# g1mv/density

Measured on NVIDIA H100. Metric: chameleon_encode_input_GBps, higher is better.
Workload: dtype u32

## Files before the change

### density_b200/csrc/chameleon_encode.cu

```cuda
#include <cstdio>
#include "common.cuh"
#include "encode_internal.cuh"

namespace dns {
namespace cham {

constexpr int TILE_Q = 4096;
__device__ __forceinline__ bool bit_test(const uint32_t* bm, uint32_t i) { return (bm[i >> 5] >> (i & 31)) & 1u; }

constexpr int F6_THREADS = 512, F6_QPT = 8;
constexpr int F6_NW = F6_THREADS / 32, F6_WQ = 32 * F6_QPT;
static_assert(F6_THREADS * F6_QPT == TILE_Q, "tile geometry");
constexpr int F6_MB_SLOTS = 4096, F6_MB_CAP = 4;
constexpr int F6_SEC_SLOTS = 64, F6_SEC_CAP = 16;
#ifdef DNS_PHASE_TIMING
__device__ long long g_f6_ph[8];
#define F6_PH(k) { if (threadIdx.x == 0 && blockIdx.x == 77) { long long tn = clock64(); g_f6_ph[k] += tn - f6_tprev; f6_tprev = tn; } }
#define F6_PH_DECL long long f6_tprev = clock64();
#else
#define F6_PH(k)
#define F6_PH_DECL
#endif
constexpr uint32_t F6_TOUCHED = 1u << 12, F6_DROPPED = 1u << 13;
struct Flag6Smem {
// ... 211 lines not shown
                const uint32_t n = (S.mbcnt[buf][slot >> 2] >> ((slot & 3u) * 8u)) & 0xFFu;
                const uint2 e2 = *reinterpret_cast<const uint2*>(&S.mb[slot][0]);
                const uint32_t me = ((hh >> 12) << 12) | myidx;
                int best = -1;
#pragma unroll
                for (int t = 0; t < F6_MB_CAP; ++t) {
                    const uint32_t e = ((t & 2) ? e2.y : e2.x) >> ((t & 1) * 16) & 0xFFFFu;
                    if ((uint32_t)t < n && ((e ^ me) >> 12) == 0) {
                        if (e < me) best = max(best, (int)(e & 0xFFFu));
                        later |= e > me;
                    }
                }
                if (n > (uint32_t)F6_MB_CAP) {
                    const uint32_t s2 = slot & (F6_SEC_SLOTS - 1);
                    const uint32_t n2 = S.seccnt[buf][s2];
                    const uint32_t mine = (hh << 12) | myidx;
                    #pragma unroll 1
                    for (uint32_t t4 = 0; t4 < n2; t4 += 4) {
                        const uint4 e4 = *reinterpret_cast<const uint4*>(&S.sec[s2][t4]);
                        const uint32_t ev[4] = {e4.x, e4.y, e4.z, e4.w};
#pragma unroll
                        for (int t = 0; t < 4; ++t) {
                            const uint32_t e = ev[t];
                            if (t4 + t < n2 && ((e ^ mine) & 0xFFFFF000u) == 0) {
                                if (e < mine) best = max(best, (int)(e & 0xFFFu));
                                later |= e > mine;
                            }
                        }
                    }
                }
                if (best >= 0) hit = (S.rec[best].x >> 16) == ff;
                else if (r.y & F6_TOUCHED) hit = (r.y >> 16) == ff;
                else unres = true;
                if (!later) {
                    S.tab[hh] = (uint16_t)ff;
                    if (ff == 0) atomicOr(&S.vbit[hh >> 5], 1u << (hh & 31));
                }
                if (hit) atomicOr(&S.sigw[buf][pos >> 5], 1u << (pos & 31));
            }
            f6_append_unres(unres, run_q0 + pos, r.x, &S.unres_count, unres_run);
        }
    }
    __syncthreads();
    F6_PH(3)
}

__global__ void __launch_bounds__(F6_THREADS, 1)
cham_flag_pass6(const uint32_t* __restrict__ in, uint64_t nquads, uint32_t tiles_total, uint32_t nruns,
                uint32_t* __restrict__ sigw_g, uint2* __restrict__ unres, uint32_t* __restrict__ unres_count,
                uint32_t* __restrict__ final_tab, const uint8_t* __restrict__ copymap, const Status* __restrict__ gate)
{
    if (gate && !(gate->nonquiet && !gate->converged)) return;
    extern __shared__ __align__(16) unsigned char smem_raw[];
    Flag6Smem& S = *reinterpret_cast<Flag6Smem*>(smem_raw);
    const uint32_t tid = threadIdx.x, lane = tid & 31, warp = tid >> 5;
    const uint32_t run = blockIdx.x;
    const uint64_t t_begin = (uint64_t)run * tiles_total / nruns;
    const uint64_t t_end = (uint64_t)(run + 1) * tiles_total / nruns;
    uint2* __restrict__ unres_run = unres + (size_t)run * 65536;
    const uint32_t pos0 = warp * F6_WQ + lane;
    const uint32_t ntile_run = (uint32_t)(t_end - t_begin);
    const uint64_t q_begin = t_begin * TILE_Q;
    const uint64_t q_end64 = (t_end * TILE_Q < nquads) ? t_end * TILE_Q : nquads;
    const uint32_t run_quads = q_begin < q_end64 ? (uint32_t)(q_end64 - q_begin) : 0u;
    const uint32_t* __restrict__ rin = in + q_begin;
    uint32_t* __restrict__ rsig = sigw_g + t_begin * (TILE_Q / 32);
    const uint8_t* __restrict__ rcm = copymap ? copymap + t_begin * 64 : nullptr;
    {
        const uint4 z = make_uint4(0, 0, 0, 0);
        uint4* t4 = reinterpret_cast<uint4*>(S.tab);
        #pragma unroll 1
        for (uint32_t i = tid; i < 65536 * 2 / 16; i += F6_THREADS) t4[i] = z;
        #pragma unroll 1
        for (uint32_t i = tid; i < 2048; i += F6_THREADS) S.vbit[i] = 0;
        #pragma unroll 1
        for (uint32_t i = tid; i < F6_MB_SLOTS / 4; i += F6_THREADS) { S.mbcnt[0][i] = 0; S.mbcnt[1][i] = 0; }
        if (tid < F6_SEC_SLOTS) { S.seccnt[0][tid] = 0; S.seccnt[1][tid] = 0; }
        if (tid == 0) { S.unres_count = 0; S.overflow = 0; }
    }
    __syncthreads();
    uint32_t nxt[F6_QPT], nxt2[F6_QPT];
#pragma unroll
    for (int j = 0; j < F6_QPT; ++j) {
        nxt[j] = (pos0 + 32 * j < run_quads) ? ld_stream_u32(rin + pos0 + 32 * j) : 0u;
        nxt2[j] = (TILE_Q + pos0 + 32 * j < run_quads) ? ld_stream_u32(rin + TILE_Q + pos0 + 32 * j) : 0u;
    }
    #pragma unroll 1
    for (uint32_t lt = 0; lt < ntile_run; ++lt) {
        uint32_t q[F6_QPT];
        const uint32_t run_q0 = lt * TILE_Q;
        const uint32_t left = run_q0 < run_quads ? run_quads - run_q0 : 0u;
        const uint32_t buf = lt & 1u;
#pragma unroll
        for (int j = 0; j < F6_QPT; ++j) { q[j] = nxt[j]; nxt[j] = nxt2[j]; }
        {
            const uint32_t nleft = left > 2u * TILE_Q ? left - 2u * TILE_Q : 0u;
            const uint32_t* __restrict__ np = rin + run_q0 + 2 * TILE_Q + pos0;
            if (nleft >= (uint32_t)TILE_Q) {
#pragma unroll
                for (int j = 0; j < F6_QPT; ++j) nxt2[j] = ld_stream_u32(np + 32 * j);
            } else {
#pragma unroll
                for (int j = 0; j < F6_QPT; ++j) nxt2[j] = (pos0 + 32 * j < nleft) ? ld_stream_u32(np + 32 * j) : 0u;
            }
        }
        if (left >= (uint32_t)TILE_Q && !rcm) {
            f6_tile<false>(S, q, (1u << F6_QPT) - 1u, buf, run_q0, unres_run);
        } else {
            uint32_t validmask = 0, cp = 0;
            if (rcm) {
#pragma unroll
                for (int b = 0; b < F6_WQ / 64; ++b) cp |= (rcm[lt * 64 + warp * (F6_WQ / 64) + b] ? 1u : 0u) << b;
            }
#pragma unroll
            for (int j = 0; j < F6_QPT; ++j)
                if (pos0 + 32 * j < left && !((cp >> (j >> 1)) & 1u)) validmask |= 1u << j;
            f6_tile<true>(S, q, validmask, buf, run_q0, unres_run);
        }
        if (tid < TILE_Q / 32) rsig[lt * (TILE_Q / 32) + tid] = S.sigw[buf][tid];
        if (tid == 0) S.overflow = 0;
    }
    #pragma unroll 1
    for (uint32_t i = tid; i < 65536; i += F6_THREADS) {
        const uint32_t v = S.tab[i];
        const uint32_t tch = (v != 0 || bit_test(S.vbit, i)) ? 0x10000u : 0u;
        final_tab[(size_t)run * 65536 + i] = v | tch;
    }
    if (tid == 0) unres_count[run] = S.unres_count < 65536u ? S.unres_count : 65536u;
#ifdef DNS_PHASE_TIMING
    if (tid == 0 && run == 77 && ntile_run) { const long long nt = ntile_run;
        printf("f6 run %u tiles %lld cycles/tile: A %lld B %lld C+deposit %lld D+S4 %lld  overflow tiles %lld dirty/tile %lld\n", run, nt, g_f6_ph[0] / nt, g_f6_ph[1] / nt,
               g_f6_ph[2] / nt, g_f6_ph[3] / nt, g_f6_ph[6], g_f6_ph[7] / nt);
        for (int k = 0; k < 8; ++k) g_f6_ph[k] = 0; }
#endif
}

__device__ __forceinline__ bool gate_open(const Status* g) { return !g || (g->nonquiet && !g->converged); }

__global__ void cham_carry_scan(const uint32_t* __restrict__ final_tab, const uint32_t* __restrict__ init, int init_untouched,
                                uint32_t nruns, uint32_t* __restrict__ carry, uint32_t* __restrict__ table_out,
                                const Status* __restrict__ gate = nullptr) {
    if (!gate_open(gate)) return;
    uint32_t hb = blockIdx.x * blockDim.x + threadIdx.x;
    if (hb >= 65536) return;
    uint32_t c = init ? init[hb] : ((hb == 0 && !init_untouched) ? 0x10000u : 0u);
    for (uint32_t r = 0; r < nruns; ++r) {
        if (carry) carry[(size_t)r * 65536 + hb] = c;
        uint32_t v = final_tab[(size_t)r * 65536 + hb];
        if (v & 0x10000u) c = v;
    }
    if (table_out) table_out[hb] = c;
}

__global__ void cham_resolve(const uint2* __restrict__ unres, const uint32_t* __restrict__ unres_count,
                             const uint32_t* __restrict__ carry, uint32_t tiles_total, uint32_t nruns,
                             uint32_t* __restrict__ sigw_g, const Status* __restrict__ gate = nullptr) {
    if (!gate_open(gate)) return;
    const uint32_t run = blockIdx.y;
    const uint32_t n = unres_count[run];
    const uint64_t run_q0 = ((uint64_t)run * tiles_total / nruns) * TILE_Q;
    for (uint32_t i = blockIdx.x * blockDim.x + threadIdx.x; i < n; i += gridDim.x * blockDim.x) {
        uint2 e = unres[(size_t)run * 65536 + i];
        uint32_t c = carry[(size_t)run * 65536 + (e.y & 0xFFFFu)];
        if ((c & 0x10000u) && (c & 0xFFFFu) == (e.y >> 16)) {
            uint64_t gq = run_q0 + e.x;
            atomicOr(&sigw_g[gq >> 5], 1u << (gq & 31));
        }
    }
}

struct ProtSmem {
    uint16_t tab[65536];
    uint32_t vbit[2048];
};

__global__ void __launch_bounds__(1024, 1)
cham_protected_pass(const uint32_t* __restrict__ in, uint64_t nbytes, const Status* __restrict__ status, int only_if_nonquiet,
                    uint32_t* __restrict__ sigw_g, uint8_t* __restrict__ copymap) {
    if (only_if_nonquiet && !(status->nonquiet && !status->converged)) return;
    extern __shared__ __align__(16) unsigned char smem_raw[];
    ProtSmem& S = *reinterpret_cast<ProtSmem*>(smem_raw);
    const uint32_t tid = threadIdx.x, lane = tid & 31;
    {
        uint4 z = make_uint4(0, 0, 0, 0);
        uint4* t4 = reinterpret_cast<uint4*>(S.tab);
        for (uint32_t i = tid; i < 65536 * 2 / 16; i += blockDim.x) t4[i] = z;
        for (uint32_t i = tid; i < 2048; i += blockDim.x) S.vbit[i] = (i == 0) ? 1u : 0u;
    }
    __syncthreads();
    if (tid >= 32) return;

    const uint64_t nquads = nbytes / 4;
    const uint64_t nblocks = (nbytes + 255) / 256;
    Protection ps; ps.init();
    uint32_t n0 = 0, n1 = 0;
    if (nblocks) {
        if (lane < nquads) n0 = in[lane];
        if (32 + lane < nquads) n1 = in[32 + lane];
    }
    for (uint64_t b = 0; b < nblocks; ++b) {
        const uint32_t q0 = n0, q1 = n1;
        {
            uint64_t g = (b + 1) * 64 + lane;
            n0 = (b + 1 < nblocks && g < nquads) ? in[g] : 0u;
            n1 = (b + 1 < nblocks && g + 32 < nquads) ? in[g + 32] : 0u;
        }
        const uint64_t bq0 = b * 64;
        const uint32_t nq = (uint32_t)((nquads - bq0 < 64) ? (nquads - bq0) : 64);
        if (ps.revert_to_copy()) {
            if (lane == 0) { copymap[b] = 1; sigw_g[2 * b] = 0; sigw_g[2 * b + 1] = 0; }
            ps.decay();
            continue;
        }
        uint32_t sig[2];
#pragma unroll
        for (int half = 0; half < 2; ++half) {
            const uint32_t q = half ? q1 : q0;
            const bool valid = half * 32 + lane < nq;
            const uint32_t p = hash_prod(q);
            uint32_t hh = valid ? prod_hash(p) : 0x10000u + lane;
            const uint32_t ff = prod_fp(p, q);
            uint32_t cur = 0; bool touched = false;
            if (valid) { cur = S.tab[hh]; touched = cur != 0 || bit_test(S.vbit, hh); }
            const uint32_t grp = __match_any_sync(0xFFFFFFFFu, hh);
            const uint32_t lower = grp & lanemask_lt();
            const int pl = lower ? 31 - __clz(lower) : 0;
            const uint32_t fprev = __shfl_sync(0xFFFFFFFFu, ff, pl);
            const bool hit = valid && (lower ? (fprev == ff) : (touched && cur == ff));
            const bool is_last = (grp & lanemask_gt()) == 0;
            if (valid && is_last && (lower || !hit)) {
                S.tab[hh] = (uint16_t)ff;
                if (ff == 0) atomicOr(&S.vbit[hh >> 5], 1u << (hh & 31));
            }
            sig[half] = __ballot_sync(0xFFFFFFFFu, hit);
            __syncwarp();
        }
        if (lane == 0) { copymap[b] = 0; sigw_g[2 * b] = sig[0]; sigw_g[2 * b + 1] = sig[1]; }
        const uint32_t hits = __popc(sig[0]) + __popc(sig[1]);
        const uint32_t tailb = (b == nblocks - 1) ? (uint32_t)(nbytes & 3) : 0u;
        const uint32_t out_sz = 8 + 4 * nq - 2 * hits + tailb;
        ps.update(out_sz >= 256);
    }
}

constexpr int PSEG = 256;

__device__ __forceinline__ uint32_t prot_pack(const Protection& ps) { return ps.copy_penalty | (ps.copy_penalty_start << 8) | (ps.previous_incompressible << 16); }
__device__ __forceinline__ void prot_walk(Protection& ps, const uint8_t* __restrict__ inc, uint64_t b0, uint64_t b1, uint8_t* __restrict__ cm) {
    for (uint64_t b = b0; b < b1; ++b) {
        if (ps.revert_to_copy()) { cm[b] = 1; ps.decay(); }
        else { cm[b] = 0; ps.update(__ldcg(&inc[b]) != 0); }
    }
}
constexpr int PROT_ROUNDS = 48, PROT_FAST_ROUNDS = 4;
constexpr int PI_THREADS = 1024;

constexpr uint32_t PC_NS = 10, PC_NP = 10, PC_NC = 2 * PC_NS * PC_NP, PC_ESC = 0xFFFFu, PC_GROUP = 128;
__host__ __device__ __forceinline__ size_t prot_table_elems(uint64_t nseg) {
    const uint64_t ngrp = (nseg + PC_GROUP - 1) / PC_GROUP;
    return (size_t)(2 * (ngrp + 2) + nseg * PC_NC + ngrp * PC_NC + 64);
}
__device__ __forceinline__ void pc_decode(uint32_t c, Protection& ps) {
    ps.copy_penalty = c % PC_NP; ps.copy_penalty_start = (c / PC_NP) % PC_NS + 1u; ps.previous_incompressible = c / (PC_NP * PC_NS);
}
__device__ __forceinline__ uint32_t pc_encode(const Protection& ps) {
    if (ps.copy_penalty >= PC_NP || ps.copy_penalty_start < 1u || ps.copy_penalty_start > PC_NS) return PC_ESC;
    return (ps.previous_incompressible * PC_NS + (ps.copy_penalty_start - 1u)) * PC_NP + ps.copy_penalty;
}

__device__ __forceinline__ void grid_barrier(unsigned int* counter, unsigned int nctas, unsigned int& epoch) {
    __syncthreads();
    if (threadIdx.x == 0) {
        __threadfence();
        atomicAdd(counter, 1u);
        const unsigned int target = (epoch + 1) * nctas;
        while (atomicAdd(counter, 0u) < target) { __nanosleep(64); }
        __threadfence();
    }
    ++epoch;
    __syncthreads();
}

__device__ unsigned long long g_prot_dbg[16][2];

__global__ void __launch_bounds__(PI_THREADS)
prot_iterate(const uint32_t* __restrict__ sigw_g, uint64_t nbytes, uint64_t nblocks, uint32_t nseg, Status* __restrict__ st, int it,
             uint8_t* __restrict__ inc, uint8_t* __restrict__ cm_old, uint8_t* __restrict__ cm_new,
             uint32_t* __restrict__ in_state, uint32_t* __restrict__ out_state, uint16_t* __restrict__ ptab) {
    if (!gate_open(st)) return;
    __shared__ uint32_t s_state[1024], s_in[1024];
    __shared__ uint8_t s_inc[PSEG], s_cm[PSEG];
    __shared__ uint32_t s_cur, s_redo;
    const uint32_t tid = threadIdx.x;
    const uint64_t gtid = (uint64_t)blockIdx.x * PI_THREADS + tid, gsz = (uint64_t)gridDim.x * PI_THREADS;
    unsigned int epoch = 0;
    unsigned int* bar = &st->barrier[it & 7];

    if (sigw_g)
        for (uint64_t b = gtid; b < nblocks; b += gsz)
            if (!(it && cm_old[b])) inc[b] = (nbytes - b * 256 >= 256) && (__popc(sigw_g[2 * b]) + __popc(sigw_g[2 * b + 1]) <= 4);
    if (gtid == 0) { st->relax_changed[0] = 0; st->relax_changed[1] = 0; st->iter_changed = 0; st->pad2[0] = 0; }
    if (gtid < 16 && it == 0) { g_prot_dbg[gtid][0] = ~0ull; g_prot_dbg[gtid][1] = 0; }
    grid_barrier(bar, gridDim.x, epoch);

    bool settled = false;
    int round = 0;
    for (int phase = 0; phase < 2 && !settled; ++phase) {
    const int limit = (phase == 0 && ptab) ? PROT_FAST_ROUNDS : PROT_ROUNDS;
    for (; round < limit; ++round) {
        for (uint64_t s = gtid; s < nseg; s += gsz) {
            const uint32_t new_in = (s && round) ? __ldcg(&out_state[s - 1]) : (1u << 8);
            if (round > 0 && new_in == in_state[s]) continue;
            Protection ps;
            ps.copy_penalty = new_in & 0xFFu; ps.copy_penalty_start = (new_in >> 8) & 0xFFu; ps.previous_incompressible = (new_in >> 16) & 1u;
            ps.counter = s * PSEG;
            const uint64_t b1 = ((s + 1) * PSEG < nblocks) ? (s + 1) * PSEG : nblocks;
            prot_walk(ps, inc, s * PSEG, b1, cm_new);
            in_state[s] = new_in;
            out_state[s] = prot_pack(ps);
// ... 494 lines not shown
    while (k < nb) {
        const uint32_t k1 = (k + 16 < nb) ? k + 16 : nb;
        for (; k < k1; ++k) { if (p.revert_to_copy()) p.decay(); else p.update(s_inc[k] != 0); }
        if (tid == 0) s_ref = prot_pack(p);
        __syncthreads();
        if (__syncthreads_and(prot_pack(p) == s_ref)) break;
    }
    if (k < nb) {
        if (tid == 0) {
            for (; k < nb; ++k) { if (p.revert_to_copy()) p.decay(); else p.update(s_inc[k] != 0); }
            s_ref = pc_encode(p);
        }
        __syncthreads();
        if (tid < PC_NC) T[(size_t)seg * PC_NC + tid] = (uint16_t)s_ref;
    } else if (tid < PC_NC) {
        T[(size_t)seg * PC_NC + tid] = (uint16_t)pc_encode(p);
    }
    __syncthreads();
    }
}

__global__ void cham_prot_groups_k(uint32_t nseg, const Status* __restrict__ st, const uint16_t* __restrict__ T, uint16_t* __restrict__ GT) {
    if (!gate_open(st)) return;
    const uint32_t ngrp = (nseg + PC_GROUP - 1) / PC_GROUP;
    const uint64_t idx = (uint64_t)blockIdx.x * blockDim.x + threadIdx.x;
    if (idx >= (uint64_t)ngrp * PC_NC) return;
    const uint32_t g = (uint32_t)(idx / PC_NC);
    uint32_t x = (uint32_t)(idx % PC_NC);
    const uint32_t s1 = ((g + 1) * PC_GROUP < nseg) ? (g + 1) * PC_GROUP : nseg;
    for (uint32_t s = g * PC_GROUP; s < s1 && x != PC_ESC; ++s) x = T[(size_t)s * PC_NC + x];
    GT[idx] = (uint16_t)x;
}
__global__ void cham_prot_transfer_k(uint32_t nseg, const Status* __restrict__ st, const uint16_t* __restrict__ GT, uint32_t* __restrict__ out) {
    if (!gate_open(st)) return;
    const uint32_t c = threadIdx.x;
    if (c >= PC_NC) return;
    const uint32_t ngrp = (nseg + PC_GROUP - 1) / PC_GROUP;
    uint32_t x = c;
    for (uint32_t g = 0; g < ngrp && x != PC_ESC; ++g) x = GT[(size_t)g * PC_NC + x];
    out[c] = x;
}

__global__ void cham_prot_enter_k(const uint32_t* __restrict__ all_transfers, uint32_t rank, uint32_t nseg, const Status* __restrict__ st,
                                  const uint16_t* __restrict__ GT, uint32_t* __restrict__ gin, ProtShard* __restrict__ ps,
                                  uint32_t* __restrict__ words) {
    if (threadIdx.x || blockIdx.x) return;
    const bool open = gate_open(st);
    words[0] = 0; words[1] = 0; words[2] = open ? 0u : 1u; words[3] = 0;
    if (!open) return;
    uint32_t x = 0;
    for (uint32_t r = 0; r < rank && x != PC_ESC; ++r) x = all_transfers[(size_t)r * PC_NC + x];
    ps->in_state = x;
    const uint32_t ngrp = (nseg + PC_GROUP - 1) / PC_GROUP;
    for (uint32_t g = 0; g < ngrp; ++g) { gin[g] = x; if (x != PC_ESC) x = GT[(size_t)g * PC_NC + x]; }
    gin[ngrp] = x;
    if (x == PC_ESC) words[1] = 1;
}
__global__ void cham_prot_seams_k(uint32_t nseg, const Status* __restrict__ st, const uint16_t* __restrict__ T, const uint32_t* __restrict__ gin,
                                  uint32_t* __restrict__ in_state) {
    if (!gate_open(st)) return;
    const uint32_t ngrp = (nseg + PC_GROUP - 1) / PC_GROUP;
    const uint32_t g = blockIdx.x * blockDim.x + threadIdx.x;
    if (g >= ngrp || gin[ngrp] == PC_ESC) return;
    uint32_t x = gin[g];
    const uint32_t s1 = ((g + 1) * PC_GROUP < nseg) ? (g + 1) * PC_GROUP : nseg;
    for (uint32_t s = g * PC_GROUP; s < s1; ++s) { in_state[s] = x; x = T[(size_t)s * PC_NC + x]; }
}
__global__ void cham_prot_walk_k(uint64_t nblocks, uint32_t nseg, const Status* __restrict__ st, int it, int warm, const uint8_t* __restrict__ inc,
                                 const uint8_t* __restrict__ cm_old, uint8_t* __restrict__ cm_new, const uint32_t* __restrict__ in_state,
                                 const uint32_t* __restrict__ gin, ProtShard* __restrict__ ps, uint32_t* __restrict__ words) {
    if (!gate_open(st)) return;
    const uint32_t ngrp = (nseg + PC_GROUP - 1) / PC_GROUP;
    const uint32_t s = blockIdx.x * blockDim.x + threadIdx.x;
    if (s >= nseg || gin[ngrp] == PC_ESC) return;
    Protection p; pc_decode(in_state[s], p);
    const uint64_t b0 = (uint64_t)s * PSEG, b1 = (b0 + PSEG < nblocks) ? b0 + PSEG : nblocks;
    p.counter = ps->first_block + b0;
    prot_walk(p, inc, b0, b1, cm_new);
    uint32_t nd = 0;
    for (uint64_t b = b0; b < b1; ++b) nd += cm_new[b] != ((it || warm) ? cm_old[b] : 0);
    if (nd) {
        atomicAdd(&words[0], nd);
        if (it < 16) atomicAdd(&ps->changed[it], nd);
    }
}

__device__ __forceinline__ void prot_round_verdict(const uint32_t* all_words, uint32_t world, uint32_t stride, bool& changed, bool& esc) {
    changed = false; esc = false;
    for (uint32_t r = 0; r < world; ++r) { changed |= all_words[stride * r] != 0; esc |= all_words[stride * r + 1] != 0; }
}
__global__ void cham_prot_commit_k(const uint32_t* __restrict__ all_words, uint32_t world, uint32_t stride, uint64_t nblocks, const Status* __restrict__ st,
                                   int it, uint8_t* __restrict__ cm_old, const uint8_t* __restrict__ cm_new) {
    if (!gate_open(st)) return;
    bool changed, esc;
    prot_round_verdict(all_words, world, stride, changed, esc);
    if (esc || !(changed || it == 0)) return;
    for (uint64_t b = (uint64_t)blockIdx.x * blockDim.x + threadIdx.x; b < nblocks; b += (uint64_t)gridDim.x * blockDim.x) cm_old[b] = cm_new[b];
}
__global__ void cham_prot_verdict_k(const uint32_t* __restrict__ all_words, uint32_t world, uint32_t stride, Status* __restrict__ st, int it,
                                    ProtShard* __restrict__ ps) {
    if (threadIdx.x || blockIdx.x || !gate_open(st)) return;
    bool changed, esc;
    prot_round_verdict(all_words, world, stride, changed, esc);
    if (esc) { ps->esc = 1; st->converged = 1; }
    else if (!changed) { ps->settled = 1; ps->rounds = (uint32_t)it + 1; st->converged = 1; }
}
__global__ void cham_prot_finish_k(Status* __restrict__ st, const ProtShard* __restrict__ ps) {
    if (threadIdx.x || blockIdx.x) return;
    if (!ps->settled || !ps->stage_ok) st->error = PROT_REFUSED;
}
__global__ void cham_prot_seam_words_k(uint64_t nblocks, const Status* __restrict__ st, uint64_t* __restrict__ d_out_size, uint32_t* __restrict__ words) {
    if (threadIdx.x || blockIdx.x) return;
    const uint64_t sz = (nblocks && !st->error) ? *d_out_size : 0;
    *d_out_size = sz;
    words[0] = 0; words[1] = 0; words[2] = st->error ? 1u : 0u; words[3] = nblocks ? 1u : 0u;
    words[4] = (uint32_t)sz; words[5] = (uint32_t)(sz >> 32); words[6] = 0; words[7] = 0;
}

}

using namespace cham;

size_t cham_workspace_bytes(size_t nbytes, int nruns_max, ChamLayout* L) {
    const uint64_t nblocks = (nbytes + 255) / 256;
    const uint64_t ntiles = (nblocks + 63) / 64;
    const uint64_t ngroups = (ntiles + SCAN_G - 1) / SCAN_G;
    size_t off = 0;
    auto take = [&](size_t bytes) { size_t o = off; off += (bytes + 255) & ~(size_t)255; return o; };
    L->status = take(sizeof(Status));
    L->sigw = take((ntiles * 64 * 2 + 64 + 256) * sizeof(uint32_t));
    L->copymap = take(ntiles * 64 + 64 + 128);
    L->copymap2 = take(ntiles * 64 + 64 + 128);
    L->seg_state = take(prot_state_bytes(ntiles * 64 / PSEG + 2));
    L->incb = take(ntiles * 64 + 64);
    L->tile_bytes = take((ntiles + 1) * sizeof(uint32_t));
    L->tile_local = take((ntiles + 1) * sizeof(uint32_t));
    L->group_total = take((ngroups + 1) * sizeof(uint64_t));
    L->group_off = take((ngroups + 1) * sizeof(uint64_t));
    L->unres = take((size_t)nruns_max * 65536 * sizeof(uint2));
    L->unres_count = take((size_t)nruns_max * sizeof(uint32_t));
    L->final_tab = take((size_t)nruns_max * 65536 * sizeof(uint32_t));
    L->carry = take((size_t)nruns_max * 65536 * sizeof(uint32_t));
    L->total = off;
    return off;
}

static cudaError_t set_smem_attrs_once() {
    static bool done = false;
    static cudaError_t err = cudaSuccess;
    if (!done) {
        err = cudaFuncSetAttribute(cham_flag_pass6, cudaFuncAttributeMaxDynamicSharedMemorySize, (int)sizeof(Flag6Smem));
        if (err == cudaSuccess)
            err = cudaFuncSetAttribute(cham_protected_pass, cudaFuncAttributeMaxDynamicSharedMemorySize, (int)sizeof(ProtSmem));
        done = true;
    }
    return err;
}

static cudaError_t prot_iterate_coop(int ctas, cudaStream_t stream, const uint32_t* sigw, uint64_t nbytes, uint64_t nblocks, uint32_t nseg, Status* st, int it,
                                     uint8_t* inc, uint8_t* cm_old, uint8_t* cm_new, uint32_t* in_state, uint32_t* out_state, uint16_t* ptab) {
    void* args[] = {&sigw, &nbytes, &nblocks, &nseg, &st, &it, &inc, &cm_old, &cm_new, &in_state, &out_state, &ptab};
    return cudaLaunchCooperativeKernel(reinterpret_cast<const void*>(prot_iterate), dim3((unsigned)ctas), dim3(PI_THREADS), args, 0, stream);
}

cudaError_t prot_debug_read(unsigned long long* out32) { return cudaMemcpyFromSymbol(out32, g_prot_dbg, sizeof(unsigned long long) * 32); }

size_t prot_state_bytes(uint64_t nseg_max) { return (2 * (nseg_max + 2) + 64) * sizeof(uint32_t) + prot_table_elems(nseg_max) * sizeof(uint16_t); }

uint32_t cham_pick_runs(size_t nbytes, int num_sms) {
    const uint64_t nblocks = (nbytes + 255) / 256;
    const uint64_t ntiles = (nblocks + 63) / 64;
    uint64_t r = ntiles / 16;
    if (r < 1) r = 1;
    if (r > (uint64_t)num_sms) r = num_sms;
    return (uint32_t)r;
}

struct ChamBufs {
    size_t nbytes; uint64_t nquads, nblocks; uint32_t ntiles, ngroups, nseg, ngrp;
    Status* st; uint32_t* sigw; uint8_t *copymap, *copymap2, *incb; uint32_t *seg_state, *tile_bytes, *tile_local; uint64_t *group_total, *group_off;
    uint2* unres; uint32_t *unres_count, *final_tab, *carry;
    uint32_t *in_state, *out_state, *gin; uint16_t *ptab, *T, *GT;
    template <class X> static X* at(uint8_t* ws, size_t off) { return reinterpret_cast<X*>(ws + off); }
    ChamBufs(uint8_t* ws, const ChamLayout& L, size_t n) {
        nbytes = n; nquads = n / 4; nblocks = (n + 255) / 256;
        ntiles = (uint32_t)((nblocks + 63) / 64); ngroups = (ntiles + SCAN_G - 1) / SCAN_G;
        nseg = (uint32_t)((nblocks + PSEG - 1) / PSEG); ngrp = (nseg + PC_GROUP - 1) / PC_GROUP;
        st = at<Status>(ws, L.status); sigw = at<uint32_t>(ws, L.sigw);
        copymap = ws + L.copymap; copymap2 = ws + L.copymap2; incb = ws + L.incb;
        seg_state = at<uint32_t>(ws, L.seg_state);
        tile_bytes = at<uint32_t>(ws, L.tile_bytes); tile_local = at<uint32_t>(ws, L.tile_local);
        group_total = at<uint64_t>(ws, L.group_total); group_off = at<uint64_t>(ws, L.group_off);
        unres = at<uint2>(ws, L.unres); unres_count = at<uint32_t>(ws, L.unres_count);
        final_tab = at<uint32_t>(ws, L.final_tab); carry = at<uint32_t>(ws, L.carry);
        in_state = seg_state; out_state = seg_state + (nseg + 1);
        ptab = reinterpret_cast<uint16_t*>(seg_state + 2 * (nseg + 1));
        gin = reinterpret_cast<uint32_t*>(ptab); T = ptab + 2 * (ngrp + 2); GT = T + (size_t)nseg * PC_NC;
    }
};

static void launch_flag_pass(const ChamBufs& B, const uint8_t* d_in, uint32_t nruns, const uint8_t* copymap, const Status* gate, cudaStream_t stream,
                             uint64_t* launches) {
    cham_flag_pass6<<<nruns, F6_THREADS, sizeof(Flag6Smem), stream>>>(reinterpret_cast<const uint32_t*>(d_in), B.nquads, B.ntiles, nruns, B.sigw, B.unres,
                                                                      B.unres_count, B.final_tab, copymap, gate);
    ++*launches;
}
static void launch_carry_resolve(const ChamBufs& B, uint32_t nruns, const uint32_t* d_carry_in, const Status* gate, cudaStream_t stream,
                                 uint64_t* launches) {
    cham_carry_scan<<<65536 / 256, 256, 0, stream>>>(B.final_tab, d_carry_in, 0, nruns, B.carry, nullptr, gate);
    cham_resolve<<<dim3(32, nruns), 256, 0, stream>>>(B.unres, B.unres_count, B.carry, B.ntiles, nruns, B.sigw, gate);
    *launches += 2;
}
static void launch_export_fold(const ChamBufs& B, uint32_t nruns, uint32_t* d_table_out, const Status* gate, cudaStream_t stream, uint64_t* launches) {
    cham_carry_scan<<<65536 / 256, 256, 0, stream>>>(B.final_tab, nullptr, 1, nruns, nullptr, d_table_out, gate);
    ++*launches;
}
static cudaError_t sizes_scan_emit(const ChamBufs& B, const uint8_t* d_in, const uint8_t* copymap, int use_copymap_if_nonquiet, bool al16_ok,
                                   uint8_t* d_out, size_t cap, uint64_t* d_out_size, cudaStream_t stream, uint64_t* launches, cudaEvent_t* ev) {
    if (copymap) {
        cham_tile_sizes<<<(B.ntiles + 7) / 8, 256, 0, stream>>>(B.sigw, copymap, B.nbytes, B.nblocks, B.ntiles, use_copymap_if_nonquiet, 0, 0, B.st, B.tile_bytes);
        ++*launches;
    }
    cudaError_t e = scan_tiles_launch(B.tile_bytes, B.ntiles, B.tile_local, B.group_total, B.group_off, B.ngroups, B.st, (uint64_t)cap, d_out_size, stream);
    if (e != cudaSuccess) return e;
    *launches += 2;
    if (ev) cudaEventRecord(ev[2], stream);
    const uint32_t* in32 = reinterpret_cast<const uint32_t*>(d_in);
    if (al16_ok && (reinterpret_cast<uintptr_t>(d_in) & 15u) == 0)
        cham_emit<true><<<B.ntiles, EM_THREADS, 0, stream>>>(in32, B.nbytes, B.nblocks, B.sigw, copymap, use_copymap_if_nonquiet, B.st, B.tile_local, B.group_off, d_out);
    else
        cham_emit<false><<<B.ntiles, EM_THREADS, 0, stream>>>(in32, B.nbytes, B.nblocks, B.sigw, copymap, use_copymap_if_nonquiet, B.st, B.tile_local, B.group_off, d_out);
    ++*launches;
    if (ev) cudaEventRecord(ev[3], stream);
    return cudaGetLastError();
}

cudaError_t cham_encode_phase1(const uint8_t* d_in, size_t nbytes, uint8_t* ws, const ChamLayout& L, uint32_t nruns,
                               uint32_t* d_table_out, cudaStream_t stream, uint64_t* launches, cudaEvent_t* ev) {
    cudaError_t e = set_smem_attrs_once();
    if (e != cudaSuccess) return e;
    const ChamBufs B(ws, L, nbytes);
    e = cudaMemsetAsync(B.st, 0, sizeof(Status), stream);
    if (e == cudaSuccess) e = cudaMemsetAsync(&B.st->first_nonquiet_block, 0xFF, sizeof(unsigned long long), stream);
    if (e != cudaSuccess) return e;
    if (B.nblocks == 0) return cudaSuccess;
    if (ev) cudaEventRecord(ev[0], stream);
    launch_flag_pass(B, d_in, nruns, nullptr, nullptr, stream, launches);
    if (ev) cudaEventRecord(ev[1], stream);
    if (d_table_out) launch_export_fold(B, nruns, d_table_out, nullptr, stream, launches);
    return cudaGetLastError();
}

static cudaError_t cham_phase2_begin(const ChamBufs& B, uint32_t nruns, const uint32_t* d_carry_in, bool assume_prev_inc, cudaStream_t stream,
                                     uint64_t* launches) {
    launch_carry_resolve(B, nruns, d_carry_in, nullptr, stream, launches);
    cham_tile_sizes<<<(B.ntiles + 7) / 8, 256, 0, stream>>>(B.sigw, nullptr, B.nbytes, B.nblocks, B.ntiles, 0, 1, assume_prev_inc ? 1 : 0, B.st, B.tile_bytes);
    ++*launches;
    return cudaGetLastError();
}

static cudaError_t cham_phase2_rounds(const ChamBufs& B, const uint8_t* d_in, uint32_t nruns, const uint32_t* d_carry_in, int it_first, int it_last,
                                      bool reset_barriers, int num_sms, cudaStream_t stream, uint64_t* launches) {
    const int num_ctas = num_sms > 0 ? num_sms : 1;
    if (it_last - it_first >= 8) return cudaErrorInvalidValue;
    if (reset_barriers) {
        cudaError_t e = cudaMemsetAsync(B.st->barrier, 0, sizeof(B.st->barrier), stream);
        if (e != cudaSuccess) return e;
    }
    for (int it = it_first; it <= it_last; ++it) {
        if (it > 0) {
            launch_flag_pass(B, d_in, nruns, B.copymap, B.st, stream, launches);
            launch_carry_resolve(B, nruns, d_carry_in, B.st, stream, launches);
        }
        cudaError_t le = prot_iterate_coop(num_ctas, stream, B.sigw, B.nbytes, B.nblocks, B.nseg, B.st, it, B.incb, B.copymap, B.copymap2, B.in_state,
                                           B.out_state, B.ptab);
        if (le != cudaSuccess) return le;
        ++*launches;
    }
    return cudaGetLastError();
}

static cudaError_t cham_phase2_finish(const ChamBufs& B, const uint8_t* d_in, uint8_t* d_out, size_t cap, uint64_t* d_out_size, bool with_copy_map,
                                      bool inorder_fallback, cudaStream_t stream, uint64_t* launches, cudaEvent_t* ev) {
    if (with_copy_map && inorder_fallback) {
        cham_protected_pass<<<1, 1024, sizeof(ProtSmem), stream>>>(reinterpret_cast<const uint32_t*>(d_in), B.nbytes, B.st, 1, B.sigw, B.copymap);
        ++*launches;
    }
    return sizes_scan_emit(B, d_in, with_copy_map ? B.copymap : nullptr, 1, true, d_out, cap, d_out_size, stream, launches, ev);
}

static cudaError_t cham_phase2_needs_more(const ChamBufs& B, cudaStream_t stream, bool* more) {
    Status h;
    cudaError_t e = cudaMemcpyAsync(&h, B.st, sizeof h, cudaMemcpyDeviceToHost, stream);
    if (e == cudaSuccess) e = cudaStreamSynchronize(stream);
    if (e != cudaSuccess) return e;
    *more = h.nonquiet && !h.converged && !h.error;
    return cudaSuccess;
}

constexpr int PROT_ITERS = 4;

struct Phase2Opts {
    const uint32_t* d_carry_in = nullptr;
    bool assume_prev_inc = false;
    bool iterate = true;
    int max_batches = 0;
    bool inorder_walk = true;
    bool* give_up = nullptr;
    uint32_t* d_table_out = nullptr;
    cudaEvent_t* ev = nullptr;
};

static cudaError_t cham_phase2(const uint8_t* d_in, size_t nbytes, uint8_t* ws, const ChamLayout& L, uint32_t nruns, uint8_t* d_out, size_t cap,
                               uint64_t* d_out_size, const Phase2Opts& o, int num_sms, cudaStream_t stream, uint64_t* launches) {
    if (nbytes == 0) return cudaMemsetAsync(d_out_size, 0, sizeof(uint64_t), stream);
    const ChamBufs B(ws, L, nbytes);
    cudaError_t e = cham_phase2_begin(B, nruns, o.d_carry_in, o.assume_prev_inc, stream, launches);
    if (e == cudaSuccess && o.iterate) e = cham_phase2_rounds(B, d_in, nruns, o.d_carry_in, 0, PROT_ITERS, false, num_sms, stream, launches);
    bool more = false;
    const int looks = o.max_batches + (o.give_up ? 1 : 0);
    for (int batch = 0; e == cudaSuccess && batch < looks; ++batch) {
        e = cham_phase2_needs_more(B, stream, &more);
        if (e != cudaSuccess || !more || batch >= o.max_batches) break;
        e = cham_phase2_rounds(B, d_in, nruns, o.d_carry_in, 8, 15, true, num_sms, stream, launches);
    }
    if (e != cudaSuccess) return e;
    if (o.give_up && more) { *o.give_up = true; return cudaSuccess; }
    e = cham_phase2_finish(B, d_in, d_out, cap, d_out_size, o.iterate, o.inorder_walk, stream, launches, o.ev);
    if (e == cudaSuccess && o.d_table_out) {
        launch_export_fold(B, nruns, o.d_table_out, nullptr, stream, launches);
        e = cudaGetLastError();
    }
    return e;
}

cudaError_t cham_encode_phase2(const uint8_t* d_in, size_t nbytes, uint8_t* ws, const ChamLayout& L, uint32_t nruns,
                               const uint32_t* d_carry_in, uint8_t* d_out, size_t cap, uint64_t* d_out_size,
                               bool allow_protected_fallback, bool assume_prev_inc, int num_sms, cudaStream_t stream, uint64_t* launches,
                               cudaEvent_t* ev) {
    Phase2Opts o;
    o.d_carry_in = d_carry_in; o.assume_prev_inc = assume_prev_inc; o.iterate = allow_protected_fallback; o.ev = ev;
    return cham_phase2(d_in, nbytes, ws, L, nruns, d_out, cap, d_out_size, o, num_sms, stream, launches);
}

cudaError_t cham_encode_phase2_blocking(const uint8_t* d_in, size_t nbytes, uint8_t* ws, const ChamLayout& L, uint32_t nruns, uint8_t* d_out,
                                        size_t cap, uint64_t* d_out_size, int max_batches, int num_sms, cudaStream_t stream, uint64_t* launches) {
    Phase2Opts o;
    o.max_batches = max_batches;
    return cham_phase2(d_in, nbytes, ws, L, nruns, d_out, cap, d_out_size, o, num_sms, stream, launches);
}

cudaError_t cham_encode_phase2_stream(const uint8_t* d_in, size_t nbytes, uint8_t* ws, const ChamLayout& L, uint32_t nruns, const uint32_t* d_carry_in,
                                      uint8_t* d_out, size_t cap, uint64_t* d_out_size, uint32_t* d_table_out, int max_batches, int num_sms,
                                      cudaStream_t stream, uint64_t* launches, bool* ok) {
    bool gave_up = false;
    Phase2Opts o;
    o.d_carry_in = d_carry_in; o.max_batches = max_batches; o.inorder_walk = false; o.give_up = &gave_up; o.d_table_out = d_table_out;
    const cudaError_t e = cham_phase2(d_in, nbytes, ws, L, nruns, d_out, cap, d_out_size, o, num_sms, stream, launches);
    *ok = !gave_up;
    return e;
}
cudaError_t cham_quads_to_table(const uint32_t* d_quads, uint32_t* d_table, cudaStream_t stream, uint64_t* launches) {
    cham_quads_to_table_k<<<65536 / 256, 256, 0, stream>>>(d_quads, d_table);
// ... 184 lines not shown
```

Baseline: 480.8.

## Stage per-run carry table in shared memory for unresolved-entry resolution

cham_resolve now launches one 1024-thread block per run instead of a 32×nruns grid. Each block first loads that run's 64K-entry carry table, packing it into a 16-bit fingerprint array plus a touched bitmap in shared memory. It then resolves unresolved entries in batches of eight loads per thread, replacing random global carry lookups with shared-memory lookups. In exchange, every nonempty run pays a full 256KB table load even when it has few unresolved entries, and parallelism drops to one CTA per run.

```diff
diff --git a/density_b200/csrc/chameleon_encode.cu b/density_b200/csrc/chameleon_encode.cu
--- a/density_b200/csrc/chameleon_encode.cu
+++ b/density_b200/csrc/chameleon_encode.cu
@@ -387,19 +387,51 @@
     if (table_out) table_out[hb] = c;
 }
 
-__global__ void cham_resolve(const uint2* __restrict__ unres, const uint32_t* __restrict__ unres_count,
-                             const uint32_t* __restrict__ carry, uint32_t tiles_total, uint32_t nruns,
-                             uint32_t* __restrict__ sigw_g, const Status* __restrict__ gate = nullptr) {
+constexpr int RS_THREADS = 1024, RS_BATCH = 8;
+struct ResolveSmem {
+    uint16_t fp[65536];
+    uint32_t touched[2048];
+};
+__global__ void __launch_bounds__(RS_THREADS, 1)
+cham_resolve(const uint2* __restrict__ unres, const uint32_t* __restrict__ unres_count, const uint32_t* __restrict__ carry, uint32_t tiles_total,
+             uint32_t nruns, uint32_t* __restrict__ sigw_g, const Status* __restrict__ gate = nullptr) {
     if (!gate_open(gate)) return;
-    const uint32_t run = blockIdx.y;
+    extern __shared__ __align__(16) unsigned char smem_raw[];
+    ResolveSmem& S = *reinterpret_cast<ResolveSmem*>(smem_raw);
+    const uint32_t tid = threadIdx.x, lane = tid & 31;
+    const uint32_t run = blockIdx.x;
     const uint32_t n = unres_count[run];
+    if (n == 0) return;
+    const uint32_t* __restrict__ crun = carry + (size_t)run * 65536;
+#pragma unroll 4
+    for (uint32_t i4 = tid; i4 < 65536 / 4; i4 += RS_THREADS) {
+        const uint4 v = __ldg(reinterpret_cast<const uint4*>(crun) + i4);
+        *reinterpret_cast<uint2*>(&S.fp[4 * i4]) = make_uint2((v.x & 0xFFFFu) | (v.y << 16), (v.z & 0xFFFFu) | (v.w << 16));
+        uint32_t t = (((v.x >> 16) & 1u) | ((v.y >> 15) & 2u) | ((v.z >> 14) & 4u) | ((v.w >> 13) & 8u)) << ((lane & 7) * 4);
+        t |= __shfl_xor_sync(0xFFFFFFFFu, t, 1);
+        t |= __shfl_xor_sync(0xFFFFFFFFu, t, 2);
+        t |= __shfl_xor_sync(0xFFFFFFFFu, t, 4);
+        if ((lane & 7) == 0) S.touched[i4 >> 3] = t;
+    }
+    __syncthreads();
     const uint64_t run_q0 = ((uint64_t)run * tiles_total / nruns) * TILE_Q;
-    for (uint32_t i = blockIdx.x * blockDim.x + threadIdx.x; i < n; i += gridDim.x * blockDim.x) {
-        uint2 e = unres[(size_t)run * 65536 + i];
-        uint32_t c = carry[(size_t)run * 65536 + (e.y & 0xFFFFu)];
-        if ((c & 0x10000u) && (c & 0xFFFFu) == (e.y >> 16)) {
-            uint64_t gq = run_q0 + e.x;
-            atomicOr(&sigw_g[gq >> 5], 1u << (gq & 31));
+    const uint2* __restrict__ urun = unres + (size_t)run * 65536;
+    #pragma unroll 1
+    for (uint32_t i0 = 0; i0 < n; i0 += RS_THREADS * RS_BATCH) {
+        uint2 e[RS_BATCH];
+#pragma unroll
+        for (int k = 0; k < RS_BATCH; ++k) {
+            const uint32_t i = i0 + k * RS_THREADS + tid;
+            e[k] = i < n ? urun[i] : make_uint2(0, 0);
+        }
+#pragma unroll
+        for (int k = 0; k < RS_BATCH; ++k) {
+            const uint32_t i = i0 + k * RS_THREADS + tid;
+            const uint32_t h = e[k].y & 0xFFFFu;
+            if (i < n && ((S.touched[h >> 5] >> (h & 31)) & 1u) && S.fp[h] == (e[k].y >> 16)) {
+                const uint64_t gq = run_q0 + e[k].x;
+                atomicOr(&sigw_g[gq >> 5], 1u << (gq & 31));
+            }
         }
     }
 }
@@ -1200,6 +1232,8 @@
         err = cudaFuncSetAttribute(cham_flag_pass6, cudaFuncAttributeMaxDynamicSharedMemorySize, (int)sizeof(Flag6Smem));
         if (err == cudaSuccess)
             err = cudaFuncSetAttribute(cham_protected_pass, cudaFuncAttributeMaxDynamicSharedMemorySize, (int)sizeof(ProtSmem));
+        if (err == cudaSuccess)
+            err = cudaFuncSetAttribute(cham_resolve, cudaFuncAttributeMaxDynamicSharedMemorySize, (int)sizeof(ResolveSmem));
         done = true;
     }
     return err;
@@ -1256,7 +1290,8 @@
 static void launch_carry_resolve(const ChamBufs& B, uint32_t nruns, const uint32_t* d_carry_in, const Status* gate, cudaStream_t stream,
                                  uint64_t* launches) {
     cham_carry_scan<<<65536 / 256, 256, 0, stream>>>(B.final_tab, d_carry_in, 0, nruns, B.carry, nullptr, gate);
-    cham_resolve<<<dim3(32, nruns), 256, 0, stream>>>(B.unres, B.unres_count, B.carry, B.ntiles, nruns, B.sigw, gate);
+    set_smem_attrs_once();
+    cham_resolve<<<nruns, RS_THREADS, sizeof(ResolveSmem), stream>>>(B.unres, B.unres_count, B.carry, B.ntiles, nruns, B.sigw, gate);
     *launches += 2;
 }
 static void launch_export_fold(const ChamBufs& B, uint32_t nruns, uint32_t* d_table_out, const Status* gate, cudaStream_t stream, uint64_t* launches) {
```

After: 485.6 (median of 6 runs). No clear change (+1.0%).
